# rlog58/dags-vae-search

Measured on AMD Instinct MI355X. Metric: DAGs/sec VAE+predictor train step, n=12 batch 4096 per GPU, at 1 MI355X, higher is better.
Workload: dtype f32 (fwd bf16x6, bwd bf16x3 split products, fp32 accumulate); 1 GPU; synthetic_v12 DAGs (n=12, card=12, N=15 tokens), PACE-VAE train step: pack + fwd + bwd + clip_grad_norm_(1.0) + Adam(1e-4), train mode dropout 0.15; per_gpu_batch=4096, global_batch=4096, waves_per_workgroup=8, parallelism=single

## Files before the change

dags_vae_search_amd/csrc/dvs_loss.h:

```cpp
#pragma once
#include "dvs_kernels.h"
#include "dvs_wimg.h"
#include "dvs_stage.h"

constexpr int LOSS_LDN2 = 36;
struct LossLds {
    dvs_bf16 *Wa, *Wb;
    dvs_bf16 *WaT, *WbT;
    float *Wn1, *Wn2, *bn1, *bn2, *be1, *w2, *b2, *lg, *lb, *scr;
};
DVS_HD inline LossLds loss_lds(char* smem) {
    LossLds l;
    l.Wa = (dvs_bf16*)smem;
    l.Wb = l.Wa + 3 * DVS_IMG64;
    l.WaT = l.Wb + 3 * DVS_IMG64;
    l.WbT = l.WaT + 2 * DVS_IMG64;
    l.Wn1 = (float*)(l.WbT + 2 * DVS_IMG64);
    l.Wn2 = l.Wn1 + 32 * DVS_LD;
    l.bn1 = l.Wn2 + 16 * LOSS_LDN2;
    l.bn2 = l.bn1 + 32;
    l.be1 = l.bn2 + 16;
    l.w2 = l.be1 + 64;
    l.b2 = l.w2 + 64;
    l.lg = l.b2 + 16;
    l.lb = l.lg + 64;
    l.scr = l.lb + 64;
    return l;
}
inline size_t loss_lds_bytes(int nwaves, int tiles_per_wave) {
    return DvsLossImg::SIZE * sizeof(dvs_bf16) + (size_t)nwaves * tiles_per_wave * DVS_SCR * sizeof(float);
}
inline void loss_plan(DvsStagePlan& p, const LossArgs& a) {
    dvs_plan_clear(p);
    const LossLds l = loss_lds(DVS_FAKE_LDS);
    dvs_plan_seg(p, DVS_FAKE_LDS, l.Wa, (const dvs_bf16*)a.wimg + DvsLossImg::Wa, (int)DvsLossImg::SIZE);
    dvs_plan_seal(p);
}
constexpr int LOSS_CHUNKS = (int)(DvsLossImg::SIZE * sizeof(dvs_bf16) / 1024);
```

dags_vae_search_amd/csrc/k_backward_heads.hip:

```cpp
#include "dvs_backward.h"
#include "dvs_wimg.h"
#include "dvs_latent_bwd.h"
#include "dvs_loss.h"

#ifdef DVS_STAMPS
__device__ unsigned long long dvs_stamps_lossb[256 * 4 * 12];
DVS_STAMP_READER(lossb)
#endif
#define LBSTAMP(k) DVS_ACC_STAMP_AT(dvs_stamps_lossb, lst_, 4, 12, k)
__global__ __launch_bounds__(256) void k_loss_bwd(LossArgs a, DvsStagePlan plan) {
#ifdef DVS_STAMPS
    unsigned long long lst_ = __builtin_amdgcn_s_memtime();
#endif
    DVS_DYN_LDS(smem);
    const LossLds l = loss_lds(smem);
    const int N = a.dims.N, C = a.dims.C;
    dvs_stage_now<(LOSS_CHUNKS + 3) / 4>(&plan, smem);
    __syncthreads();
    const Lane L = dvs_lane();
    float* scrV = l.scr + L.wave * 3 * DVS_SCR;
    float* scrU = scrV + DVS_SCR;
    float* dlm = scrU + DVS_SCR;
    const float b2 = l.b2[0];
    const float gr = a.gcoef[0];
    f4 dWn1[2][4], dWn2[1][2], aWa[4], aWb[4], abU = f4_zero(), abV = f4_zero(), dbn1[2], dbn2[1], dw2[4], dgam[4], dbet[4];
    float db2 = 0.f;
#pragma unroll
    for (int i = 0; i < 4; ++i) dw2[i] = dgam[i] = dbet[i] = aWa[i] = aWb[i] = f4_zero();
#pragma unroll
    for (int i = 0; i < 2; ++i) {
        dbn1[i] = f4_zero();
        dWn2[0][i] = f4_zero();
#pragma unroll
        for (int j = 0; j < 4; ++j) dWn1[i][j] = f4_zero();
    }
    dbn2[0] = f4_zero();
    LBSTAMP(0);
    const dvs_bf16* const slots = (const dvs_bf16*)l.scr;
    constexpr int SLOT_STRIDE = 2 * 3 * DVS_SCR;
    for (int base = blockIdx.x * L.nwaves; base < a.dims.B; base += gridDim.x * L.nwaves) {
        const int dag = base + L.wave;
        if (dag >= a.dims.B) {
            const f4 z[4] = {f4_zero(), f4_zero(), f4_zero(), f4_zero()};
            dvs_park_bf((dvs_bf16*)scrV, z, L);
            dvs_park_bf((dvs_bf16*)scrU, z, L);
            dvs_park_bf((dvs_bf16*)dlm, z, L);
            __syncthreads();
            dvs_coop_dw_bf(aWa, abU, slots, slots + 2 * 2 * DVS_SCR, SLOT_STRIDE, L);
            dvs_coop_dw_bf(aWb, abV, slots + 2 * DVS_SCR, slots + 2 * 2 * DVS_SCR, SLOT_STRIDE, L);
            __syncthreads();
            continue;
        }
        f4 h[4], xhat[4];
        float rstd;
        dvs_load_x<true>(h, xhat, rstd, a.xin, a.ln, l.lg, l.lb, dag, N, L);
        const int nxt = dag + gridDim.x * L.nwaves;
        const float touch = a.xin[(size_t)(nxt < a.dims.B ? nxt : dag) * DVS_TILE + L.lane * 16];
        const DvsRecord* rec = a.rec + dag;
        f4 hN[4];
        dvs_t2n<4>(hN, h, scrV, L);
        LBSTAMP(1);
        f4 dh[4] = {f4_zero(), f4_zero(), f4_zero(), f4_zero()};
        {
            f4 t1p[2], t1[2];
#pragma unroll
            for (int t = 0; t < 2; ++t) t1p[t] = dvs_vecT(l.bn1, t, L);
            dvs_mat_T<2, 4>(t1p, h, l.Wn1, DVS_LD, 0, L);
#pragma unroll
            for (int t = 0; t < 2; ++t)
#pragma unroll
                for (int kk = 0; kk < 4; ++kk) t1[t][kk] = fmaxf(t1p[t][kk], 0.f);
            f4 lgt[1] = {*(const f4*)(l.bn2 + 4 * L.g)};
            dvs_mat_T<1, 2>(lgt, t1, l.Wn2, LOSS_LDN2, 0, L);
            float mx = -3.0e38f;
#pragma unroll
            for (int reg = 0; reg < 4; ++reg) mx = (4 * L.g + reg < C) ? fmaxf(mx, lgt[0][reg]) : mx;
            mx = dvs_max_g(mx);
            f4 ex;
            float se = 0.f;
#pragma unroll
            for (int reg = 0; reg < 4; ++reg) {
                ex[reg] = (4 * L.g + reg < C) ? __expf(lgt[0][reg] - mx) : 0.f;
                se += ex[reg];
            }
            se = dvs_sum_g(se);
            const float rse = dvs_rcp(se);
            const int target = rec->label[(L.r + 1) & 15];
            const bool vt = L.r < N - 1;
            f4 dlg[1];
#pragma unroll
            for (int reg = 0; reg < 4; ++reg) {
                const int c = 4 * L.g + reg;
                dlg[0][reg] = (vt && c < C) ? gr * (ex[reg] * rse - (c == target ? 1.f : 0.f)) : 0.f;
            }
            dbn2[0] += dlg[0];
            f4 dlgN[1], t1N[2];
            dvs_t2n<1>(dlgN, dlg, scrV, L);
            dvs_t2n<2>(t1N, t1, scrV, L);
            dvs_outer_acc<1, 2>(dWn2, dlgN, t1N);
            f4 dt1[2] = {f4_zero(), f4_zero()};
            dvs_mat_Tt<2, 1>(dt1, dlg, l.Wn2, LOSS_LDN2, 0, L);
#pragma unroll
            for (int t = 0; t < 2; ++t) {
#pragma unroll
                for (int kk = 0; kk < 4; ++kk) dt1[t][kk] = t1p[t][kk] > 0.f ? dt1[t][kk] : 0.f;
                dbn1[t] += dt1[t];
            }
            f4 dt1N[2];
            dvs_t2n<2>(dt1N, dt1, scrV, L);
            dvs_outer_acc<2, 4>(dWn1, dt1N, hN);
            dvs_mat_Tt<4, 2>(dh, dt1, l.Wn1, DVS_LD, 0, L);
        }
        LBSTAMP(2);
        f4 U[4], V[4], w2v[4], dU[4], dV[4];
#pragma unroll
        for (int t = 0; t < 4; ++t) {
            U[t] = f4_zero();
            V[t] = dvs_vecT(l.be1, t, L);
            w2v[t] = dvs_vecT(l.w2, t, L);
            dU[t] = dV[t] = f4_zero();
        }
        {
            const Split3T hs = dvs_split3_T(h);
            dvs_matb3<4>(U, hs, l.Wa, 64, 0, L);
            dvs_matb3<4>(V, hs, l.Wb, 64, 0, L);
        }
#pragma unroll
        for (int t = 0; t < 4; ++t) {
            *(f4*)(scrV + L.r * DVS_LD + 16 * t + 4 * L.g) = V[t];
            *(f4*)(scrU + L.r * DVS_LD + 16 * t + 4 * L.g) = U[t];
        }
        dvs_wave_sync();
        const unsigned par = rec->parents[(L.r + 1) & 15];
        LBSTAMP(3);
        f4 sU[4] = {f4_zero(), f4_zero(), f4_zero(), f4_zero()}, sV[4] = {f4_zero(), f4_zero(), f4_zero(), f4_zero()};
        for (int j0 = 0; j0 < N - 2; j0 += 2) {
            f4 pre[2][4], ev[2] = {f4_zero(), f4_zero()};
            const bool has2 = j0 + 1 < N - 2;
            const int jj[2] = {j0, has2 ? j0 + 1 : j0};
#pragma unroll
            for (int u = 0; u < 2; ++u)
#pragma unroll
                for (int t = 0; t < 4; ++t) {
                    const f4 x = U[t] + *(const f4*)(scrV + jj[u] * DVS_LD + 16 * t + 4 * L.g);
#pragma unroll
                    for (int kk = 0; kk < 4; ++kk) pre[u][t][kk] = fmaxf(x[kk], 0.f);
                    ev[u] += w2v[t] * pre[u][t];
                }
            float dl[2];
#pragma unroll
            for (int u = 0; u < 2; ++u) {
                const float logit = dvs_sum_g((ev[u][0] + ev[u][1]) + (ev[u][2] + ev[u][3])) + b2;
                const bool pv = (L.r > jj[u]) && (L.r <= N - 2) && (u == 0 || has2);
                const float truth = (float)((par >> (jj[u] + 1)) & 1u);
                const float sg = dvs_rcp(1.0f + __expf(-logit));
                dl[u] = pv ? gr * (sg - truth) : 0.f;
            }
#pragma unroll
            for (int u = 0; u < 2; ++u)
#pragma unroll
                for (int t = 0; t < 4; ++t) {
                    dw2[t] += pre[u][t] * dl[u];
                    f4 st;
#pragma unroll
                    for (int kk = 0; kk < 4; ++kk) st[kk] = fminf(fmaxf(pre[u][t][kk] * 1.0e30f, 0.f), 1.f);
                    sU[t] += st * dl[u];
                }
            if (L.g == 0) {
                db2 += dl[0] + dl[1];
                dlm[L.r * 16 + j0] = dl[0];
                if (has2) dlm[L.r * 16 + j0 + 1] = dl[1];
            }
        }
        dvs_wave_sync();
        LBSTAMP(4);
#pragma unroll 2
        for (int i = 1; i <= N - 2; ++i) {
            const float dl = (L.r < i) ? dlm[i * 16 + L.r] : 0.f;
#pragma unroll
            for (int t = 0; t < 4; ++t) {
                const f4 x = *(const f4*)(scrU + i * DVS_LD + 16 * t + 4 * L.g) + V[t];
                f4 st;
#pragma unroll
                for (int kk = 0; kk < 4; ++kk) st[kk] = fminf(fmaxf(x[kk] * 1.0e30f, 0.f), 1.f);
                sV[t] += st * dl;
            }
        }
#pragma unroll
        for (int t = 0; t < 4; ++t) {
            dU[t] = w2v[t] * sU[t];
            dV[t] = w2v[t] * sV[t];
        }
        dvs_wave_sync();
        LBSTAMP(5);
        dvs_park_bf((dvs_bf16*)scrV, dU, L);
        dvs_park_bf((dvs_bf16*)scrU, dV, L);
        dvs_park_bf((dvs_bf16*)dlm, h, L);
        __syncthreads();
        dvs_coop_dw_bf(aWa, abU, slots, slots + 2 * 2 * DVS_SCR, SLOT_STRIDE, L);
        dvs_coop_dw_bf(aWb, abV, slots + 2 * DVS_SCR, slots + 2 * 2 * DVS_SCR, SLOT_STRIDE, L);
        __syncthreads();
        LBSTAMP(6);
        dvs_matb_T<4>(dh, dvs_split_T(dU), l.WaT, l.WaT + DVS_IMG64, 0, L);
        dvs_matb_T<4>(dh, dvs_split_T(dV), l.WbT, l.WbT + DVS_IMG64, 0, L);
        dvs_ln_bwd(dh, xhat, rstd, l.lg, dgam, dbet, L);
        dvs_store_tile(a.gout, dag, dh, L);
#ifndef DVS_EMU
        asm volatile("" ::"v"(touch));
#else
        (void)touch;
#endif
        LBSTAMP(7);
    }
    __syncthreads();
    LBSTAMP(8);
    float* slab = a.slab + (size_t)blockIdx.x * a.P;
    {
        dvs_coop_flush<4>(nullptr, slab + a.o_edge0_w, aWa, L, false, false, 128);
        dvs_coop_flush<4>(nullptr, slab + a.o_edge0_w + 64, aWb, L, false, false, 128);
        if (L.r == 0) {
#pragma unroll
            for (int reg = 0; reg < 4; ++reg) slab[a.o_edge0_b + 16 * L.wave + 4 * L.g + reg] = abV[reg];
        }
        float* rN1 = (float*)smem;
        float* rN2 = rN1 + 4 * 2048;
        float* rv = rN2 + 4 * 512;
        dvs_stage_dw<2, 4>(rN1, dWn1, L);
        dvs_stage_dw<1, 2>(rN2, dWn2, L);
        float* es = rv + 192 + 4 * DVS_RED_VEC + 16 + L.wave * DVS_SCR;
        dvs_stage_vec<2>(rv, dbn1, es, L);
        dvs_stage_vec<1>(rv + 128, dbn2, es, L);
        dvs_stage_vec<4>(rv + 192 + DVS_RED_VEC, dw2, es, L);
        dvs_stage_vec<4>(rv + 192 + 2 * DVS_RED_VEC, dgam, es, L);
        dvs_stage_vec<4>(rv + 192 + 3 * DVS_RED_VEC, dbet, es, L);
        const float sb2 = dvs_sum_wave(L.g == 0 ? db2 : 0.f);
        float* rb2 = rv + 192 + 4 * DVS_RED_VEC;
        if (L.lane == 0) rb2[L.wave] = sb2;
        __syncthreads();
        dvs_flush_dw<2, 4>(rN1, slab + a.o_node0_w, L);
        dvs_flush_dw<1, 2>(rN2, slab + a.o_node2_w, L, C, 32);
        dvs_flush_vec<2>(rv, slab + a.o_node0_b, L);
        dvs_flush_vec<1>(rv + 128, slab + a.o_node2_b, L, C);
        dvs_flush_vec<4>(rv + 192 + DVS_RED_VEC, slab + a.o_edge2_w, L);
        dvs_flush_vec<4>(rv + 192 + 2 * DVS_RED_VEC, slab + a.o_ln_g, L);
        dvs_flush_vec<4>(rv + 192 + 3 * DVS_RED_VEC, slab + a.o_ln_b, L);
        if (threadIdx.x == 0) {
            float s = rb2[0];
            for (int w = 1; w < L.nwaves; ++w) s += rb2[w];
            slab[a.o_edge2_b] = s;
        }
    }
    LBSTAMP(9);
}

void dvs_launch_loss_bwd(const LossArgs& a, int grid, dvs_stream_t st) {
    const size_t lds = loss_lds_bytes(4, 3);
    DvsStagePlan plan;
    loss_plan(plan, a);
    DVS_SET_LDS(k_loss_bwd, lds);
    DVS_LAUNCH(k_loss_bwd, dim3(grid), dim3(256), lds, st, a, plan);
}

__global__ __launch_bounds__(512) void k_embed_bwd(EmbedArgs a, const float* gout2, int site2, DvsStagePlan plan) {
    DVS_DYN_LDS(smem);
    const int N = a.dims.N, C = a.dims.C;
    float* W1 = (float*)smem;
    float* W2 = W1 + 2 * DVS_MAXTOK * DVS_LD;
    float* labw = W2 + 64 * EMB_LDW2;
    float* labb = labw + 32 * 16;
    float* scr0 = labb + 32;
    if (blockDim.x >= 512) dvs_stage_now<3>(&plan, smem);
    else dvs_stage_now<5>(&plan, smem);
    __syncthreads();
    const Lane L = dvs_lane();
    const DvsDrop D = dvs_drop_of(a.dims);
    float* scr = scr0 + L.wave * DVS_SCR;
    f4 dW2[4][2], dlabb[2], dW1a[1][4], dW1b[1][4], dlab[2][1];
#pragma unroll
    for (int i = 0; i < 4; ++i) dW2[i][0] = dW2[i][1] = dW1a[0][i] = dW1b[0][i] = f4_zero();
    dlabb[0] = dlabb[1] = dlab[0][0] = dlab[1][0] = f4_zero();
    for (int dag = blockIdx.x * L.nwaves + L.wave; dag < a.dims.B; dag += gridDim.x * L.nwaves) {
        const DvsRecord* rec = a.rec + dag;
        const bool valid = L.r < N;
        const int label = rec->label[L.r];
        const uint32_t gdag = a.dims.dag_offset + dag;
        const EmbSel sel = dvs_emb_selectors(rec, N, scr, L);
        f4 e1[4];
        dvs_emb_hidden(e1, W1, N, sel, L);
        for (int src = 0; src < 2; ++src) {
            const float* gsrc = src == 0 ? a.gout : gout2;
            if (!gsrc) continue;
            const int site = src == 0 ? a.site : site2;
            f4 gx[4];
            dvs_load_grad(gx, gsrc, dag, N, L);
            f4 dle[2];
#pragma unroll
            for (int t = 0; t < 2; ++t)
#pragma unroll
                for (int kk = 0; kk < 4; ++kk) {
                    const int f = 16 * t + 4 * L.g + kk;
                    const float pre = labw[f * 16 + label] + labb[f];
                    dle[t][kk] = (valid && pre > 0.f) ? gx[t][kk] : 0.f;
                }
            dlabb[0] += dle[0];
            dlabb[1] += dle[1];
            const uint32_t k1 = dvs_site_key(a.dims.seed_lo, a.dims.seed_hi, site, gdag);
            f4 m1[4] = {f4_splat(1.f), f4_splat(1.f), f4_splat(1.f), f4_splat(1.f)};
            dvs_dropout_tile(m1, k1, D, L);
            f4 e1d[4];
#pragma unroll
            for (int t = 0; t < 4; ++t) e1d[t] = e1[t] * m1[t];
            f4 de2[2] = {gx[2], gx[3]};
            dvs_dropout_tile<2>(de2, dvs_site_key(a.dims.seed_lo, a.dims.seed_hi, site + 1, gdag), D, L);
            f4 e1dN[4], de2N[2], dleN[2];
            dvs_t2n<4>(e1dN, e1d, scr, L);
            dvs_t2n<2>(de2N, de2, scr, L);
            dvs_t2n<2>(dleN, dle, scr, L);
            dvs_outer_acc<4, 2>(dW2, e1dN, de2N);
            f4 de1[4] = {f4_zero(), f4_zero(), f4_zero(), f4_zero()};
            dvs_mat_T<4, 2>(de1, de2, W2, EMB_LDW2, 0, L);
#pragma unroll
            for (int t = 0; t < 4; ++t) de1[t] *= m1[t];
#pragma unroll
            for (int t = 0; t < 4; ++t)
#pragma unroll
                for (int kk = 0; kk < 4; ++kk) de1[t][kk] = e1[t][kk] > 0.f ? de1[t][kk] : 0.f;
            f4 de1N[4];
            dvs_t2n<4>(de1N, de1, scr, L);
            f4 selA[1] = {sel.selA}, parA[1] = {sel.parA}, labA[1] = {sel.labA};
            dvs_outer_acc<1, 4>(dW1a, selA, de1N);
            dvs_outer_acc<1, 4>(dW1b, parA, de1N);
            dvs_outer_acc<2, 1>(dlab, dleN, labA);
        }
    }
    __syncthreads();
    float* slab = a.slab + (size_t)blockIdx.x * a.P;
    float* r1a = (float*)smem;
    float* r1b = r1a + 8 * 1024;
    float* rlab = r1b + 8 * 1024;
    float* rv = rlab + 8 * 512;
    dvs_stage_dw<1, 4>(r1a, dW1a, L);
    dvs_stage_dw<1, 4>(r1b, dW1b, L);
    dvs_stage_dw<2, 1>(rlab, dlab, L);
    dvs_stage_vec<2>(rv, dlabb, rv + 8 * 32 + L.wave * DVS_SCR, L);
    __syncthreads();
    dvs_flush_dw<1, 4>(r1a, slab + a.oW1, L, N, 64);
    dvs_flush_dw<1, 4>(r1b, slab + a.oW1 + (size_t)N * 64, L, N, 64);
    dvs_flush_dw<2, 1>(rlab, slab + a.olab_w, L, 32, C, C);
    dvs_flush_vec<2>(rv, slab + a.olab_b, L);
    __syncthreads();
    float* rW2 = (float*)smem;
    dvs_stage_dw<4, 2>(rW2, dW2, L);
    __syncthreads();
    dvs_flush_dw<4, 2>(rW2, slab + a.oW2, L);
}

void dvs_launch_embed_bwd(const EmbedArgs& a, const float* gout2, int site2, int grid, int nw, dvs_stream_t st) {
    size_t lds = (2 * DVS_MAXTOK * DVS_LD + 64 * EMB_LDW2 + 32 * 16 + 32 + 8 * DVS_SCR) * 4;
    const size_t red = (8 * (1024 + 1024 + 512) + 8 * 32 + 8 * DVS_SCR) * 4;
    if (lds < red) lds = red;
    DvsStagePlan plan;
    dvs_plan_clear(plan);
    dvs_plan_seg(plan, DVS_FAKE_LDS, DVS_FAKE_LDS, a.embimg, 2 * DvsEmbImg::FLOATS);
    dvs_plan_seal(plan);
    DVS_SET_LDS(k_embed_bwd, lds);
    DVS_LAUNCH(k_embed_bwd, dim3(grid), dim3(nw == 4 ? 256 : 512), lds, st, a, gout2, site2, plan);
}

constexpr int LATB_WAVES = 8;
__global__ __launch_bounds__(64 * LATB_WAVES) void k_latent_bwd(LatentBwdArgs a) {
    __shared__ f4 part[LATB_WAVES][2][64];
    dvs_latent_bwd_group<LATB_WAVES>(a, part, (int)blockIdx.x * 16, (int)blockIdx.x * 16 + 8);
}

void dvs_launch_latent_bwd(const LatentBwdArgs& a, dvs_stream_t st) {
    const int ngroups = (a.dims.B + 15) / 16;
    DVS_LAUNCH(k_latent_bwd, dim3(ngroups), dim3(64 * LATB_WAVES), 0, st, a);
}

constexpr int FC_MT = 4;
__global__ __launch_bounds__(512) void k_fc_dw(FcDwArgs a) {
    __shared__ f4 red[4][FC_MT * 6 + 2][64];
    const Lane L = dvs_lane();
    const int B = a.dims.B, N = a.dims.N;
    const int ldw = N * 64;
    const int nmg = 16 * a.dims.NT;
    const int mg = blockIdx.x % nmg, q = blockIdx.x / nmg;
    const size_t dstride = (size_t)a.dims.NT * DVS_TILE;
    const int per_q = (B + DVS_FC_PARTS - 1) / DVS_FC_PARTS;
    const int per_w = (per_q + 7) / 8;
    const int d0 = q * per_q + L.wave * per_w;
    int d1 = d0 + per_w;
    if (d1 > (q + 1) * per_q) d1 = (q + 1) * per_q;
    if (d1 > B) d1 = B;
    f4 acc[FC_MT][4], acc3[FC_MT][2];
    f4 bs3 = f4_zero();
    f4 bsfc = f4_zero();
#pragma unroll
    for (int j = 0; j < FC_MT; ++j) {
#pragma unroll
        for (int t = 0; t < 4; ++t) acc[j][t] = f4_zero();
        acc3[j][0] = acc3[j][1] = f4_zero();
    }
    for (int c0 = d0; c0 < d1; c0 += 16) {
        float ga[4][4], zb[4][2], xb[4][FC_MT], gm[4][FC_MT], live[4];
#pragma unroll
        for (int ks = 0; ks < 4; ++ks) {
            const int d = c0 + 4 * ks + L.g;
            const bool dv = d < d1;
            const size_t dd = dv ? d : 0;
            live[ks] = dv ? 1.f : 0.f;
#pragma unroll
            for (int t = 0; t < 4; ++t) ga[ks][t] = a.gz[dd * 64 + 16 * t + L.r];
#pragma unroll
            for (int t = 0; t < 2; ++t) zb[ks][t] = a.z[dd * 32 + 16 * t + L.r];
#pragma unroll
            for (int j = 0; j < FC_MT; ++j) {
                xb[ks][j] = a.xenc[dd * dstride + 16 * (FC_MT * mg + j) + L.r];
                gm[ks][j] = a.gmem[dd * dstride + 16 * (FC_MT * mg + j) + L.r];
            }
        }
#pragma unroll
        for (int ks = 0; ks < 4; ++ks) {
#pragma unroll
            for (int t = 0; t < 4; ++t) ga[ks][t] *= live[ks];
#pragma unroll
            for (int j = 0; j < FC_MT; ++j) {
                gm[ks][j] *= live[ks];
                bs3[j] += gm[ks][j];
            }
#pragma unroll
            for (int t = 0; t < 4; ++t) bsfc[t] += ga[ks][t];
#pragma unroll
            for (int j = 0; j < FC_MT; ++j) {
#pragma unroll
                for (int t = 0; t < 4; ++t) acc[j][t] = dvs_mfma(ga[ks][t], xb[ks][j], acc[j][t]);
#pragma unroll
                for (int t = 0; t < 2; ++t) acc3[j][t] = dvs_mfma(gm[ks][j], zb[ks][t], acc3[j][t]);
            }
        }
    }
#pragma unroll
    for (int j = 0; j < FC_MT; ++j) bs3[j] = dvs_sum_g(bs3[j]);
#pragma unroll
    for (int t = 0; t < 4; ++t) bsfc[t] = dvs_sum_g(bsfc[t]);
    if (L.wave < 4) {
#pragma unroll
        for (int j = 0; j < FC_MT; ++j) {
#pragma unroll
            for (int t = 0; t < 4; ++t) red[L.wave][6 * j + t][L.lane] = acc[j][t];
            red[L.wave][6 * j + 4][L.lane] = acc3[j][0];
            red[L.wave][6 * j + 5][L.lane] = acc3[j][1];
        }
        red[L.wave][6 * FC_MT][L.lane] = bsfc;
        red[L.wave][6 * FC_MT + 1][L.lane] = bs3;
    }
    __syncthreads();
    if (L.wave >= 4) {
        const int w = L.wave - 4;
#pragma unroll
        for (int j = 0; j < FC_MT; ++j) {
#pragma unroll
            for (int t = 0; t < 4; ++t) red[w][6 * j + t][L.lane] += acc[j][t];
            red[w][6 * j + 4][L.lane] += acc3[j][0];
            red[w][6 * j + 5][L.lane] += acc3[j][1];
        }
        red[w][6 * FC_MT][L.lane] += bsfc;
        red[w][6 * FC_MT + 1][L.lane] += bs3;
    }
    __syncthreads();
    if (L.wave >= 4) return;
    const int j = L.wave;
    const int m = FC_MT * mg + j;
    f4 tot[8];
#pragma unroll
    for (int i = 0; i < 6; ++i) {
        tot[i] = red[0][6 * j + i][L.lane];
#pragma unroll
        for (int w = 1; w < 4; ++w) tot[i] += red[w][6 * j + i][L.lane];
    }
#pragma unroll
    for (int i = 0; i < 2; ++i) {
        tot[6 + i] = red[0][6 * FC_MT + i][L.lane];
#pragma unroll
        for (int w = 1; w < 4; ++w) tot[6 + i] += red[w][6 * FC_MT + i][L.lane];
    }
    float* out = a.fcpart + (size_t)q * a.P;
    const int mm = m & 63;
    {
        const int tok = 16 * (m >> 6) + 4 * (mm & 3) + (L.r >> 2);
        const int f = 16 * (mm >> 4) + 4 * ((mm >> 2) & 3) + (L.r & 3);
        if (tok < N) {
#pragma unroll
            for (int t = 0; t < 4; ++t)
#pragma unroll
                for (int reg = 0; reg < 4; ++reg) {
                    const int o = 16 * (t & 1) + 4 * L.g + reg;
                    out[(t < 2 ? a.o_fc1_w : a.o_fc2_w) + (size_t)o * ldw + tok * 64 + f] = tot[t][reg];
                }
            if (L.g == 0) {
                const float b3 = j == 0 ? tot[7][0] : j == 1 ? tot[7][1] : j == 2 ? tot[7][2] : tot[7][3];
                out[a.o_fc3_b + tok * 64 + f] = b3;
            }
        }
    }
    {
        const int tok = 16 * (m >> 6) + 4 * (mm & 3) + L.g;
        const int fb = 16 * (mm >> 4) + 4 * ((mm >> 2) & 3);
        if (tok < N) {
#pragma unroll
            for (int t = 0; t < 2; ++t)
#pragma unroll
                for (int reg = 0; reg < 4; ++reg)
                    out[a.o_fc3_w + (size_t)(tok * 64 + fb + reg) * 32 + 16 * t + L.r] = tot[4 + t][reg];
        }
    }
    if (mg == 0 && j == 0 && L.g == 0) {
#pragma unroll
        for (int t = 0; t < 4; ++t) out[(t < 2 ? a.o_fc1_b : a.o_fc2_b) + 16 * (t & 1) + L.r] = tot[6][t];
    }
}

void dvs_launch_fc_dw(const FcDwArgs& a, dvs_stream_t st) {
    DVS_LAUNCH(k_fc_dw, dim3(16 * a.dims.NT * DVS_FC_PARTS), dim3(512), 0, st, a);
}
```

Before: 3.449 million DAGs/s.

## Fold triangular edge loops across lane rows to balance loss backward work

The edge-logit loops in the loss backward kernel iterate over a triangular set of (i,j) pairs, so many lanes sat idle behind pv masks. This folds the triangle so each row r also handles its mirror row M-r's edges. That roughly halves the loop trip count, from N-2 to about (N-2)/2. Partial gradient sums for the mirrored rows are exchanged through LDS scratch, which adds extra wave syncs, extra LDS traffic and more index arithmetic per iteration.

```diff
diff --git a/dags_vae_search_amd/csrc/dvs_loss.h b/dags_vae_search_amd/csrc/dvs_loss.h
--- a/dags_vae_search_amd/csrc/dvs_loss.h
+++ b/dags_vae_search_amd/csrc/dvs_loss.h
@@ -36,4 +36,36 @@
     dvs_plan_seg(p, DVS_FAKE_LDS, l.Wa, (const dvs_bf16*)a.wimg + DvsLossImg::Wa, (int)DvsLossImg::SIZE);
     dvs_plan_seal(p);
 }
-constexpr int LOSS_CHUNKS = (int)(DvsLossImg::SIZE * sizeof(dvs_bf16) / 1024);
+constexpr int LOSS_XCH = 256;
+struct EdgeFold {
+    int H, own, tot, shift, mate, q;
+    bool gives, gets;
+};
+struct EdgeSlot {
+    int f, pos;
+    bool own, live;
+};
+__device__ __forceinline__ EdgeFold dvs_edge_fold(int M, int r, int q) {
+    EdgeFold F;
+    const bool in = r <= M;
+    const int C = M > 0 ? M >> 1 : 0;
+    F.H = M > 0 ? M - C : 0;
+    F.q = q;
+    F.gives = in && 2 * q < M;
+    F.gets = in && 2 * q > M;
+    F.own = in ? (q < C ? q : C) : 0;
+    F.tot = F.gives ? M - C : F.own;
+    F.shift = C - F.own;
+    F.mate = F.gives ? M - r : 0;
+    return F;
+}
+__device__ __forceinline__ EdgeSlot dvs_fold_slot(const EdgeFold& F, int k, int r) {
+    EdgeSlot s;
+    s.own = k < F.own;
+    s.live = k < F.tot;
+    s.f = s.live ? (s.own ? r : F.mate) : 0;
+    s.pos = s.live ? (s.own ? k : k + F.shift) : 0;
+    return s;
+}
+
+constexpr int LOSS_CHUNKS =(int)(DvsLossImg::SIZE * sizeof(dvs_bf16) / 1024);
diff --git a/dags_vae_search_amd/csrc/k_backward_heads.hip b/dags_vae_search_amd/csrc/k_backward_heads.hip
--- a/dags_vae_search_amd/csrc/k_backward_heads.hip
+++ b/dags_vae_search_amd/csrc/k_backward_heads.hip
@@ -131,30 +131,38 @@
             *(f4*)(scrU + L.r * DVS_LD + 16 * t + 4 * L.g) = U[t];
         }
         dvs_wave_sync();
-        const unsigned par = rec->parents[(L.r + 1) & 15];
+        const int M = N - 2;
+        const EdgeFold F1 = dvs_edge_fold(M, L.r, L.r), F2 = dvs_edge_fold(M, L.r, M - L.r);
+        const unsigned par_own = rec->parents[(L.r + 1) & 15], par_mate = rec->parents[(F1.mate + 1) & 15];
+        float* xch = dlm + LOSS_XCH + 4 * L.g;
         LBSTAMP(3);
         f4 sU[4] = {f4_zero(), f4_zero(), f4_zero(), f4_zero()}, sV[4] = {f4_zero(), f4_zero(), f4_zero(), f4_zero()};
-        for (int j0 = 0; j0 < N - 2; j0 += 2) {
+        f4 sX[4] = {f4_zero(), f4_zero(), f4_zero(), f4_zero()};
+        for (int k0 = 0; k0 < F1.H; k0 += 2) {
             f4 pre[2][4], ev[2] = {f4_zero(), f4_zero()};
-            const bool has2 = j0 + 1 < N - 2;
-            const int jj[2] = {j0, has2 ? j0 + 1 : j0};
-#pragma unroll
-            for (int u = 0; u < 2; ++u)
+            const EdgeSlot s[2] = {dvs_fold_slot(F1, k0, L.r), dvs_fold_slot(F1, k0 + 1, L.r)};
+#pragma unroll
+            for (int u = 0; u < 2; ++u) {
+                const float* pu = scrU + s[u].f * DVS_LD + 4 * L.g;
+                const float* pv = scrV + s[u].pos * DVS_LD + 4 * L.g;
 #pragma unroll
                 for (int t = 0; t < 4; ++t) {
-                    const f4 x = U[t] + *(const f4*)(scrV + jj[u] * DVS_LD + 16 * t + 4 * L.g);
+                    const f4 x = *(const f4*)(pu + 16 * t) + *(const f4*)(pv + 16 * t);
 #pragma unroll
                     for (int kk = 0; kk < 4; ++kk) pre[u][t][kk] = fmaxf(x[kk], 0.f);
                     ev[u] += w2v[t] * pre[u][t];
                 }
-            float dl[2];
+            }
+            float dl[2], dlo[2], dlx[2];
 #pragma unroll
             for (int u = 0; u < 2; ++u) {
                 const float logit = dvs_sum_g((ev[u][0] + ev[u][1]) + (ev[u][2] + ev[u][3])) + b2;
-                const bool pv = (L.r > jj[u]) && (L.r <= N - 2) && (u == 0 || has2);
-                const float truth = (float)((par >> (jj[u] + 1)) & 1u);
+                const unsigned par = s[u].own ? par_own : par_mate;
+                const float truth = (float)((par >> (s[u].pos + 1)) & 1u);
                 const float sg = dvs_rcp(1.0f + __expf(-logit));
-                dl[u] = pv ? gr * (sg - truth) : 0.f;
+                dl[u] = s[u].live ? gr * (sg - truth) : 0.f;
+                dlo[u] = s[u].own ? dl[u] : 0.f;
+                dlx[u] = s[u].own ? 0.f : dl[u];
             }
 #pragma unroll
             for (int u = 0; u < 2; ++u)
@@ -164,27 +172,62 @@
                     f4 st;
 #pragma unroll
                     for (int kk = 0; kk < 4; ++kk) st[kk] = fminf(fmaxf(pre[u][t][kk] * 1.0e30f, 0.f), 1.f);
-                    sU[t] += st * dl[u];
+                    sU[t] += st * dlo[u];
+                    sX[t] += st * dlx[u];
                 }
             if (L.g == 0) {
                 db2 += dl[0] + dl[1];
-                dlm[L.r * 16 + j0] = dl[0];
-                if (has2) dlm[L.r * 16 + j0 + 1] = dl[1];
-            }
+                if (s[0].live) dlm[s[0].f * 16 + s[0].pos] = dl[0];
+                if (s[1].live) dlm[s[1].f * 16 + s[1].pos] = dl[1];
+            }
+        }
+        if (F1.gives) {
+#pragma unroll
+            for (int t = 0; t < 4; ++t) *(f4*)(xch + 64 * F1.q + 16 * t) = sX[t];
+        }
+        dvs_wave_sync();
+        if (F1.gets) {
+#pragma unroll
+            for (int t = 0; t < 4; ++t) sU[t] += *(const f4*)(xch + 64 * (M - F1.q) + 16 * t);
         }
         dvs_wave_sync();
         LBSTAMP(4);
-#pragma unroll 2
-        for (int i = 1; i <= N - 2; ++i) {
-            const float dl = (L.r < i) ? dlm[i * 16 + L.r] : 0.f;
-#pragma unroll
-            for (int t = 0; t < 4; ++t) {
-                const f4 x = *(const f4*)(scrU + i * DVS_LD + 16 * t + 4 * L.g) + V[t];
-                f4 st;
-#pragma unroll
-                for (int kk = 0; kk < 4; ++kk) st[kk] = fminf(fmaxf(x[kk] * 1.0e30f, 0.f), 1.f);
-                sV[t] += st * dl;
-            }
+#pragma unroll
+        for (int t = 0; t < 4; ++t) sX[t] = f4_zero();
+        for (int k0 = 0; k0 < F2.H; k0 += 2) {
+            const EdgeSlot s[2] = {dvs_fold_slot(F2, k0, L.r), dvs_fold_slot(F2, k0 + 1, L.r)};
+            float dlo[2], dlx[2];
+            f4 x[2][4];
+#pragma unroll
+            for (int u = 0; u < 2; ++u) {
+                const int i = s[u].f + 1 + s[u].pos;
+                const float dl = s[u].live ? dlm[i * 16 + s[u].f] : 0.f;
+                dlo[u] = s[u].own ? dl : 0.f;
+                dlx[u] = s[u].own ? 0.f : dl;
+                const float* pu = scrU + i * DVS_LD + 4 * L.g;
+                const float* pv = scrV + s[u].f * DVS_LD + 4 * L.g;
+#pragma unroll
+                for (int t = 0; t < 4; ++t) x[u][t] = *(const f4*)(pu + 16 * t) + *(const f4*)(pv + 16 * t);
+            }
+#pragma unroll
+            for (int u = 0; u < 2; ++u)
+#pragma unroll
+                for (int t = 0; t < 4; ++t) {
+                    f4 st;
+#pragma unroll
+                    for (int kk = 0; kk < 4; ++kk) st[kk] = fminf(fmaxf(x[u][t][kk] * 1.0e30f, 0.f), 1.f);
+                    sV[t] += st * dlo[u];
+                    sX[t] += st * dlx[u];
+                }
+        }
+        if (F2.gives) {
+#pragma unroll
+            for (int t = 0; t < 4; ++t) *(f4*)(xch + 64 * F2.q + 16 * t) = sX[t];
+        }
+        dvs_wave_sync();
+        if (F2.gets) {
+#pragma unroll
+            for (int t = 0; t < 4; ++t) sV[t] += *(const f4*)(xch + 64 * (M - F2.q) + 16 * t);
         }
 #pragma unroll
         for (int t = 0; t < 4; ++t) {
```

Result: no change. 3.460 million DAGs/s, median of 6 (+0.3%).
